# ruanyyyyyyy/point-cloud-process

Hardware: AMD Instinct MI355X
Metric: correspondence-pairs/sec + ms/ICP-iter, 120k-pt KITTI pair (higher is better)
Workload: dtype f64; 1 GPU; point-to-point ICP iteration, 120000 x 120000 KITTI-shaped synthetic scan pair per GPU (BASELINE configs[1]); exact 1-NN via grid; nn=grid, pairs_per_gpu=1, points_src=120000, points_tgt=120000

## Files before the change

### point-cloud-process_amd/csrc/pcr_grid_search.hip

```cpp
#include <atomic>
#include <chrono>
#include <cmath>
#include <cstdlib>
#include <cstring>
#include "pcr_descent.h"
#include "pcr_icp_step.h"

constexpr unsigned int HARD_SCAN_T = 192;
constexpr int HARD_STACK = 160;
constexpr long long ID_NONE = 0x7fffffffffffffffll;
constexpr int H_NLIST = 32;
constexpr int H_CSTRIDE = 32;
__host__ __device__ static inline unsigned int hard_list_cap(long long nq) {
    const long long halves = (nq + 15) / 16;
    return (unsigned int)(((halves + H_NLIST - 1) / H_NLIST) * 16 + 64);
}

template <int G>
__device__ static inline void group_best(double& bd2, long long& bid, unsigned int& bpos) {
#pragma unroll
    for (int off = G / 2; off > 0; off >>= 1) {
        const double od2 = __shfl_xor(bd2, off, 64);
        const long long oid = __shfl_xor(bid, off, 64);
        const unsigned int opos = __shfl_xor(bpos, off, 64);
// ... 33 lines not shown
    unsigned int c_start[WT_MAXC];
    unsigned int c_off[WT_MAXC + 1];
    unsigned short own[WT_PR];
};

__device__ static inline unsigned int wave_incl_scan_max(unsigned int v) {
    v = max(v, dpp_u32<0x111, 0xf>(0u, v));
    v = max(v, dpp_u32<0x112, 0xf>(0u, v));
    v = max(v, dpp_u32<0x114, 0xf>(0u, v));
    v = max(v, dpp_u32<0x118, 0xf>(0u, v));
    v = max(v, dpp_u32<0x142, 0xa>(0u, v));
    v = max(v, dpp_u32<0x143, 0xc>(0u, v));
    return v;
}

__device__ static inline int row16_min(int v) {
    v = min(v, __builtin_amdgcn_update_dpp(0, v, 0xb1, 0xf, 0xf, true));
    v = min(v, __builtin_amdgcn_update_dpp(0, v, 0x4e, 0xf, 0xf, true));
    v = min(v, __builtin_amdgcn_update_dpp(0, v, 0x141, 0xf, 0xf, true));
    v = min(v, __builtin_amdgcn_update_dpp(0, v, 0x140, 0xf, 0xf, true));
    return v;
}
__device__ static inline int row16_max(int v) {
    v = max(v, __builtin_amdgcn_update_dpp(0, v, 0xb1, 0xf, 0xf, true));
    v = max(v, __builtin_amdgcn_update_dpp(0, v, 0x4e, 0xf, 0xf, true));
    v = max(v, __builtin_amdgcn_update_dpp(0, v, 0x141, 0xf, 0xf, true));
    v = max(v, __builtin_amdgcn_update_dpp(0, v, 0x140, 0xf, 0xf, true));
    return v;
}

struct wt_xyz { double x, y, z; };

__device__ static inline wt_xyz ld_xyz_global(const void* p) {
    const __attribute__((address_space(1))) double* g = (const __attribute__((address_space(1))) double*)reinterpret_cast<const double*>(p);
    return wt_xyz{g[0], g[1], g[2]};
}

template <typename T>
__device__ static inline const T* as_global(const T* p) {
    return (const T*)(const __attribute__((address_space(1))) T*)p;
}

struct wt_state {
    double ax, ay, az;
    long long qi;
    float bound2;
    unsigned int cand_pos;
    unsigned int won;
    bool open, clamped, qvalid;
    unsigned int staged;
    unsigned long long dbg_pairs;
    unsigned int dbg_passes;
    unsigned long long probe;
};

struct wt_pre {
    pcr_pt p;
    unsigned int seed_pos;
    wt_xyz seed_b;
};
__device__ __forceinline__ static void wtile_preload(const unsigned int tile, const int lane, const pcr_pt* __restrict__ q, const long long nq,
                                                     const unsigned int* __restrict__ res_pos, const wt_xyz* __restrict__ prev_xyz, wt_pre& P) {
    const long long qi = (long long)tile * WT_Q + (lane & (WT_Q - 1));
    P.seed_pos = POS_NONE;
    P.seed_b = wt_xyz{0.0, 0.0, 0.0};
    P.p.x = P.p.y = P.p.z = 0.0; P.p.id = 0;
    if (qi < nq) {
        if (prev_xyz) {
            P.seed_pos = res_pos[qi];
            P.seed_b = prev_xyz[qi];
        }
        P.p = q[qi];
    }
}

#ifndef PCR_WT_WAVES
#define PCR_WT_WAVES 4
#endif
__device__ __forceinline__ static void wtile_search(const pcr_grid_view& gv, wtile_lds* L, const unsigned int tile, const int lane, const wt_pre& P,
                                                    pcr_pt* __restrict__ q, const long long nq, const pcr_xform& x, const int has_x, const int write_back,
                                                    const double max_d2, const int gated, const unsigned int pcap, unsigned int* __restrict__ res_pos,
                                                    double* __restrict__ res_d2, unsigned long long* __restrict__ dbg,
                                                    const wt_xyz* __restrict__ prev_xyz, wt_state& S, const unsigned long long* probe_p = nullptr,
                                                    const unsigned int probe_stride = 0, const unsigned int probe_groups = 0, const unsigned int probe_total = 0) {
    typedef float f4 __attribute__((ext_vector_type(4)));
    const pcr_pt* __restrict__ g_pts = as_global(gv.pts);
#ifdef PCR_WT_DIAG
    const unsigned long long t_start = dbg ? __builtin_amdgcn_s_memtime() : 0;
    unsigned long long t_ph[8] = {0, 0, 0, 0, 0, 0, 0, 0}, t_last = t_start;
#define WT_STAMP(i) do { if (dbg) { const unsigned long long t_now = __builtin_amdgcn_s_memtime(); t_ph[i] += t_now - t_last; t_last = t_now; } } while (0)
#define WT_WHY(v) do { why = (v); } while (0)
    int why = 0;
#else
#define WT_STAMP(i) do {} while (0)
#define WT_WHY(v) do {} while (0)
#endif
    const long long qi = (long long)tile * WT_Q + (lane & (WT_Q - 1));
    const bool qvalid = qi < nq;
    double ax = 0, ay = 0, az = 0;
    bool clamped = false;
    const unsigned int seed_pos = P.seed_pos;
    const wt_xyz seed_b = P.seed_b;
    if (qvalid) {
        const pcr_pt p = P.p;
        ax = p.x; ay = p.y; az = p.z;
        if (has_x) {
            xform_apply(x, p, &ax, &ay, &az);
            if (write_back && lane < WT_Q) {
                pcr_pt o;
                o.x = ax; o.y = ay; o.z = az; o.id = p.id;
                q[qi] = o;
            }
        }
        cell_coord(ax, gv.lo[0], gv.inv_cell0, &clamped);
        cell_coord(ay, gv.lo[1], gv.inv_cell0, &clamped);
        cell_coord(az, gv.lo[2], gv.inv_cell0, &clamped);
    }
    
    WT_STAMP(0);
    bool open = qvalid;
    const float gate2 = gated ? (float)max_d2 * (1.0f + 1e-6f) : INFINITY;
    float bound2 = gate2;
    unsigned int cand_pos = POS_NONE, won = POS_NONE;
    if (prev_xyz && qvalid && !clamped) {
        const unsigned int pp = seed_pos;
        if (pp != POS_NONE) {
            const wt_xyz b = seed_b;
            const double dx = ax - b.x, dy = ay - b.y, dz = az - b.z;
            const float up = (float)((dx * dx + dy * dy) + dz * dz) * (1.0f + 2e-7f) + 1e-37f;
            if (up < bound2) { bound2 = up; cand_pos = pp; }
        }
    }
    unsigned long long dbg_pairs = 0, probe_v = 0;
    unsigned int dbg_passes = 0, staged = 0;
    const int max_passes = prev_xyz ? WT_PASSES_SEEDED : WT_PASSES;
    unsigned int staged_done = 0;
    float ring = 1.0f;
#pragma unroll 1
    for (int pass = 0; pass < max_passes; ++pass) {
        const bool part = open && !clamped;
        if (!__any(part)) break;
        if (pass > 0 && staged_done > (unsigned int)WT_HEAVY_STOP) break;
        int mn[3], mx[3];
        {
            const float rho = (cand_pos != POS_NONE) ? sqrtf(bound2) * (1.0f + 1e-6f) : fminf((float)gv.cell0 * ring, sqrtf(gate2));
            const double rc = fmin((double)rho * gv.inv_cell0, 262144.0);
            const double tx = (ax - gv.lo[0]) * gv.inv_cell0, ty = (ay - gv.lo[1]) * gv.inv_cell0, tz = (az - gv.lo[2]) * gv.inv_cell0;
            const int cmax = (int)PCR_COORD_MAX;
            mn[0] = part ? max(0, min(cmax, (int)floor(tx - rc) + (int)PCR_COORD_BIAS)) : 0x7fffffff;
            mx[0] = part ? max(0, min(cmax, (int)floor(tx + rc) + (int)PCR_COORD_BIAS)) : -1;
            mn[1] = part ? max(0, min(cmax, (int)floor(ty - rc) + (int)PCR_COORD_BIAS)) : 0x7fffffff;
            mx[1] = part ? max(0, min(cmax, (int)floor(ty + rc) + (int)PCR_COORD_BIAS)) : -1;
            mn[2] = part ? max(0, min(cmax, (int)floor(tz - rc) + (int)PCR_COORD_BIAS)) : 0x7fffffff;
            mx[2] = part ? max(0, min(cmax, (int)floor(tz + rc) + (int)PCR_COORD_BIAS)) : -1;
        }
#pragma unroll
        for (int k = 0; k < 3; ++k) {
            int lo_k = row16_min(mn[k]), hi_k = row16_max(mx[k]);
            lo_k = min(__builtin_amdgcn_readlane(lo_k, 0), __builtin_amdgcn_readlane(lo_k, 16));
            hi_k = max(__builtin_amdgcn_readlane(hi_k, 0), __builtin_amdgcn_readlane(hi_k, 16));
            mn[k] = __builtin_amdgcn_readfirstlane(lo_k);
            mx[k] = __builtin_amdgcn_readfirstlane(hi_k);
        }
        int level = -1, blo0 = 0, blo1 = 0, blo2 = 0, d0 = 0, d1 = 0, d2 = 0;
        const int n_levels = gv.levels;
        for (int l = 0; l < n_levels; ++l) {
            const int b0 = mn[0] >> (2 * l), b1 = mn[1] >> (2 * l), b2 = mn[2] >> (2 * l);
            const int e0 = (mx[0] >> (2 * l)) - b0 + 1, e1 = (mx[1] >> (2 * l)) - b1 + 1, e2 = (mx[2] >> (2 * l)) - b2 + 1;
            if (e0 > WT_MAXC || e1 > WT_MAXC || e2 > WT_MAXC || e0 * e1 > WT_MAXC || e0 * e1 * e2 > WT_MAXC) continue;
            const int n0 = ((b0 + e0 - 1) >> 1) - (b0 >> 1) + 1, n1 = ((b1 + e1 - 1) >> 1) - (b1 >> 1) + 1, n2 = ((b2 + e2 - 1) >> 1) - (b2 >> 1) + 1;
            if (n0 * n1 * n2 > 64) continue;
            level = l; blo0 = b0; blo1 = b1; blo2 = b2; d0 = e0; d1 = e1; d2 = e2;
            break;
        }
        level = __builtin_amdgcn_readfirstlane(level);
        if (level < 0) { if (part) WT_WHY(1); break; }
        blo0 = __builtin_amdgcn_readfirstlane(blo0); blo1 = __builtin_amdgcn_readfirstlane(blo1); blo2 = __builtin_amdgcn_readfirstlane(blo2);
        d0 = __builtin_amdgcn_readfirstlane(d0); d1 = __builtin_amdgcn_readfirstlane(d1); d2 = __builtin_amdgcn_readfirstlane(d2);
        ++dbg_passes;
        WT_STAMP(1);
        unsigned int ncell = 0;
        bool big_child = false;
        {
            const int lim = (int)(PCR_COORD_MAX >> (2 * level));
            const int bx0 = blo0 >> 1, by0 = blo1 >> 1, bz0 = blo2 >> 1;
            const int nb0 = ((blo0 + d0 - 1) >> 1) - bx0 + 1, nb1 = ((blo1 + d1 - 1) >> 1) - by0 + 1, nb2 = ((blo2 + d2 - 1) >> 1) - bz0 + 1;
            const int nb01 = nb0 * nb1, nblk = nb01 * nb2;
            pcr_block_slot e;
            bool have = false;
            int BX = 0, BY = 0, BZ = 0;
            if (lane < nblk) {
                int iz = (int)((float)lane * __builtin_amdgcn_rcpf((float)nb01));
                iz -= (iz * nb01 > lane);
                iz += ((iz + 1) * nb01 <= lane);
                const int rem = lane - iz * nb01;
                int iy = (int)((float)rem * __builtin_amdgcn_rcpf((float)nb0));
                iy -= (iy * nb0 > rem);
                iy += ((iy + 1) * nb0 <= rem);
                const int ix = rem - iy * nb0;
                BX = bx0 + ix; BY = by0 + iy; BZ = bz0 + iz;
                const int blim = lim >> 1;
                if (BX >= 0 && BY >= 0 && BZ >= 0 && BX <= blim && BY <= blim && BZ <= blim)
                    have = lookup_block(as_global(gv.btable[level]), gv.bmask[level], (unsigned int)BX, (unsigned int)BY, (unsigned int)BZ, &e);
// ... 465 lines not shown
        const double cell = gv.cell0 * (double)(1ll << (2 * top));
        const int b0 = (int)(PCR_COORD_BIAS >> (2 * top));
        bool valid = lane < 8;
        const unsigned int X = b0 + (lane & 1), Y = b0 + ((lane >> 1) & 1), Z = b0 + ((lane >> 2) & 1);
        unsigned int s = 0, e = 0;
        double bdist = 0.0;
        if (valid) {
            bdist = box_dist2(gv, top, cell, X, Y, Z, ax, ay, az);
            valid = bdist <= bound2 && lookup_cell(gv.table[top], gv.mask[top], X, Y, Z, &s, &e);
        }
        hard_disperse(gv, L, sp, lane, valid, s, e, X, Y, Z, top, bdist, ax, ay, az, bd2, bid, bpos, bound2, h_pts, bw);
        ++h_steps;
        hard_drain(gv, L, sp, lane, ax, ay, az, bd2, bid, bpos, bound2, h_steps, h_pts, bw);
    }
    {
        const double m = wave_min_f64(bd2);
        unsigned long long cm = __ballot(bpos != POS_NONE && bd2 == m);
        if (!cm) { bd2 = DBL_MAX; bid = ID_NONE; bpos = POS_NONE; if (win) { win[0] = win[1] = win[2] = 0.0; } return; }
        int wl = (int)__ffsll((long long)cm) - 1;
        cm &= cm - 1;
        if (cm) {
            long long best_id = readlane_i64(bid, wl);
            while (cm) {
                const int l = (int)__ffsll((long long)cm) - 1;
                cm &= cm - 1;
                const long long id_l = readlane_i64(bid, l);
                if (id_l < best_id) { best_id = id_l; wl = l; }
            }
        }
        bd2 = m;
        bid = readlane_i64(bid, wl);
        bpos = (unsigned int)__builtin_amdgcn_readlane((int)bpos, wl);
        if (win) {
#pragma unroll
            for (int k = 0; k < 3; ++k)
                win[k] = readlane_f64(bw[k], wl);
        }
    }
}

__global__ void __launch_bounds__(256)
grid_hard_kernel(pcr_grid_view gv, const work_item* __restrict__ list, const unsigned int* __restrict__ count_p, long long nq, double max_d2, int gated,
                 unsigned int* __restrict__ res_pos, double* __restrict__ res_d2, unsigned long long* __restrict__ dbg,
                 const pcr_icp_dev_state* __restrict__ st) {
    __shared__ hard_lds s_lds[4];
    if (st && st->stop) return;
    const int lane = threadIdx.x & 63, wave = threadIdx.x >> 6;
    hard_lds* L = &s_lds[wave];
    unsigned int l_cnt = lane < H_NLIST ? count_p[H_CSTRIDE * lane] : 0u;
    unsigned int l_inc = l_cnt;
#pragma unroll
    for (int off = 1; off < H_NLIST; off <<= 1) {
        const unsigned int o = __shfl_up(l_inc, off, 64);
        if (lane >= off) l_inc += o;
    }
    const unsigned int count = __shfl(l_inc, H_NLIST - 1, 64);
    const unsigned int l_exc = l_inc - l_cnt;
    const unsigned int l_cap = hard_list_cap(nq);
    for (unsigned int w = blockIdx.x * 4 + wave; w < count; w += gridDim.x * 4) {
        const int hl = (int)__ffsll((long long)__ballot(lane < H_NLIST && l_exc <= w && w < l_exc + l_cnt)) - 1;
        const work_item it = list[(size_t)hl * l_cap + (w - __shfl(l_exc, hl, 64))];
        const unsigned long long h_t0 = dbg ? __builtin_amdgcn_s_memtime() : 0;
        unsigned int h_steps = 0, h_pts = 0;
        int s_level0 = 0;
        double bd2;
        long long bid;
        unsigned int bpos;
        hard_search(gv, L, lane, it.ax, it.ay, it.az, gated ? fmin(it.best_d2, max_d2) : it.best_d2, it.best_pos != POS_NONE, bd2, bid, bpos, h_steps,
                    h_pts, s_level0);
        if (lane == 0) {
            res_pos[it.qi] = bpos;
            if (res_d2) res_d2[it.qi] = bd2;
            if (dbg && w < 60000) {
                dbg[(1 << 17) + w * 4 + 0] = __builtin_amdgcn_s_memtime() - h_t0;
                dbg[(1 << 17) + w * 4 + 1] = ((unsigned long long)h_steps << 32);
                dbg[(1 << 17) + w * 4 + 2] = h_pts;
                dbg[(1 << 17) + w * 4 + 3] = (unsigned long long)(it.best_pos != POS_NONE) | ((unsigned long long)(s_level0 + 1) << 8);
            }
        }
    }
}

constexpr int ACC_SETS = 32;
constexpr int PASS_GROUPS = 32;
constexpr int PASS_SYNC_STRIDE = 32;
constexpr int PASS_SYNC_WORDS = PASS_SYNC_STRIDE * (PASS_GROUPS + 1);
constexpr unsigned long long ITEM_NONE = ~0ull;
constexpr unsigned int POISON_HI = 0xfffffffeu;
__device__ static inline unsigned long long item_poison(unsigned int pass_id) { return ((unsigned long long)POISON_HI << 32) | pass_id; }
#ifndef PCR_PASS_SPIN_LIMIT
#define PCR_PASS_SPIN_LIMIT (1u << 21)
#endif
constexpr unsigned int PASS_SPIN_LIMIT = PCR_PASS_SPIN_LIMIT;
constexpr int Q_BITS = 22;
constexpr unsigned long long Q_MASK = (1ull << Q_BITS) - 1ull;
constexpr long long PASS_MAX_NQ = 1ll << 26;
struct pass_args {
    unsigned long long* items;
    unsigned long long* sync;
    unsigned int cap;
    unsigned long long* acc;
    wt_xyz* prev_xyz;
    double scale, inv_scale;
    pcr_icp_dev_state* st;
    pcr_icp_loop_args la;
    unsigned int* tile_cost;
    unsigned int pass_id;
    unsigned long long* host_block;
    unsigned int notify;
    unsigned int* plog;
};
constexpr int PASS_LOG_WORDS = 3 * PCR_ICP_MAX_LOG + 8;
constexpr size_t HOST_LOG_OFF = (sizeof(pcr_icp_dev_state) + 63) & ~(size_t)63;
constexpr size_t HOST_FLAG_OFF = 8192 - 8;
static_assert(HOST_LOG_OFF + 4 * PASS_LOG_WORDS <= HOST_FLAG_OFF, "state + pass log + flag fit the landing block");
__host__ __device__ static inline unsigned int pass_item_cap(long long nq) {
    const long long tiles = (nq + WT_Q - 1) / WT_Q + 4;
    return (unsigned int)(((tiles + PASS_GROUPS - 1) / PASS_GROUPS) * (WT_Q + 1));
}

__device__ static inline long long to_fixed(double v, double scale) {
    constexpr double BIG = 6755399441055744.0;
    return __double_as_longlong(__builtin_fma(v, scale, BIG)) - __double_as_longlong(BIG);
}

__device__ static inline void acc_fixed_add(unsigned long long* __restrict__ acc, unsigned int set, int lane, double mk, double scale) {
    if (lane < PCR_NMOM - 1 && mk != 0.0)
        atomicAdd(acc + (size_t)(set % ACC_SETS) * PCR_NMOM + lane, (unsigned long long)to_fixed(mk, scale));
}

__device__ static inline void acc_fixed_add_ll(unsigned long long* __restrict__ acc, unsigned int set, int lane, long long v) {
    if (lane < PCR_NMOM - 1 && v != 0) atomicAdd(acc + (size_t)(set % ACC_SETS) * PCR_NMOM + lane, (unsigned long long)v);
}

__device__ static inline unsigned long long ld_dev(const unsigned long long* p) {
    return __hip_atomic_load(p, __ATOMIC_RELAXED, __HIP_MEMORY_SCOPE_AGENT);
}
__device__ static inline void st_dev(unsigned long long* p, unsigned long long v) {
    __hip_atomic_store(p, v, __ATOMIC_RELAXED, __HIP_MEMORY_SCOPE_AGENT);
}

union pass_lds {
    wtile_lds t;
    hard_lds h;
    double xch[WT_Q * (PCR_NMOM - 1)];
    long long xll[WT_Q * (PCR_NMOM - 1)];
};

__device__ __forceinline__ static void pass_serve_item(const pcr_grid_view& gv, pass_lds* L, const int lane, const unsigned long long w, const double max_d2,
                                                       const pass_args& A, unsigned int* __restrict__ res_pos, unsigned long long* __restrict__ dbg,
                                                       const unsigned int dbg_slot, const unsigned long long t_start) {
    const unsigned int w_lo = (unsigned int)w, w_hi = (unsigned int)(w >> 32);
    const double ax = __hiloint2double(__builtin_amdgcn_readlane((int)w_hi, 0), __builtin_amdgcn_readlane((int)w_lo, 0));
    const double ay = __hiloint2double(__builtin_amdgcn_readlane((int)w_hi, 1), __builtin_amdgcn_readlane((int)w_lo, 1));
    const double az = __hiloint2double(__builtin_amdgcn_readlane((int)w_hi, 2), __builtin_amdgcn_readlane((int)w_lo, 2));
    const unsigned int qi = (unsigned int)__builtin_amdgcn_readlane((int)w_lo, 3);
    const float cand_b2 = __uint_as_float((unsigned int)__builtin_amdgcn_readlane((int)w_hi, 3));
    const unsigned long long h_t0 = dbg ? __builtin_amdgcn_s_memtime() : 0;
    unsigned int h_steps = 0, h_pts = 0;
    int s_level0 = 0;
    double bd2;
    long long bid;
    unsigned int bpos;
    const bool have_cand = cand_b2 < INFINITY;
    double win[3];
    hard_search(gv, &L->h, lane, ax, ay, az, have_cand ? fmin((double)cand_b2, max_d2) : max_d2, have_cand, bd2, bid, bpos, h_steps, h_pts, s_level0, win);
    wave_sync();
    if (bpos != POS_NONE) {
        if (lane == 0) {
            pcr_pt b;
            b.x = win[0]; b.y = win[1]; b.z = win[2]; b.id = 0;
            A.prev_xyz[qi] = wt_xyz{b.x, b.y, b.z};
            double m[PCR_NMOM];
#pragma unroll
            for (int k = 0; k < PCR_NMOM; ++k) m[k] = 0.0;
            moments_add(m, gv.origin, ax, ay, az, b, max_d2, 1);
#pragma unroll
            for (int k = 0; k < PCR_NMOM - 1; ++k) L->xch[k] = m[k];
        }
        wave_sync();
        acc_fixed_add(A.acc, qi, lane, lane < PCR_NMOM - 1 ? L->xch[lane] : 0.0, A.scale);
        wave_sync();
    }
    if (lane == 0) {
        res_pos[qi] = bpos;
        if (dbg && dbg_slot < 60000) {
            dbg[(1 << 17) + dbg_slot * 4 + 0] = __builtin_amdgcn_s_memtime() - h_t0;
            dbg[(1 << 17) + dbg_slot * 4 + 1] = ((unsigned long long)h_steps << 32) | (unsigned int)((h_t0 - t_start) >> 4);
            dbg[(1 << 17) + dbg_slot * 4 + 2] = h_pts;
            dbg[(1 << 17) + dbg_slot * 4 + 3] = (unsigned long long)have_cand | ((unsigned long long)(s_level0 + 1) << 8);
        }
    }
}

__device__ __forceinline__ static void pass_finish(const pcr_grid_view& gv, pass_lds* L, const int lane, const pass_args& A, unsigned long long* root,
                                                   unsigned long long* __restrict__ dbg) {
    constexpr int HEAD_WORDS = (int)(pcr::ICP_STATE_HEAD_BYTES / 8);
    static_assert(pcr::ICP_STATE_HEAD_BYTES % 8 == 0 && HEAD_WORDS <= 64, "state head: one word per lane");
    double* const head = L->xch + 32;
    unsigned long long hw = 0, err_w = 0;
    if (lane < HEAD_WORDS) hw = reinterpret_cast<const unsigned long long*>(A.st)[lane];
    if (lane == 63) err_w = ld_dev(root + 16);
    const int mom = lane % PCR_NMOM, part = lane / PCR_NMOM;
    long long sum = 0;
    if (part < 3) {
        constexpr int PER = (ACC_SETS + 2) / 3;
        unsigned long long v[PER];
#pragma unroll
        for (int j = 0; j < PER; ++j) {
            const int set = part + 3 * j;
            v[j] = set < ACC_SETS ? ld_dev(A.acc + (size_t)set * PCR_NMOM + mom) : 0ull;
        }
#pragma unroll
        for (int j = 0; j < PER; ++j) {
            const int set = part + 3 * j;
            if (v[j]) st_dev(A.acc + (size_t)set * PCR_NMOM + mom, 0ull);
            sum += (long long)v[j];
        }
    }
    if (dbg && lane == 0) dbg[(1 << 19) - 4] = __builtin_amdgcn_s_memrealtime();
    sum += __shfl(sum, lane + PCR_NMOM, 64) + __shfl(sum, lane + 2 * PCR_NMOM, 64);
    wave_sync();
    if (dbg && lane == 0) dbg[(1 << 19) - 3] = __builtin_amdgcn_s_memrealtime();
    if (lane < PCR_NMOM) L->xch[lane] = (double)sum * A.inv_scale;
    if (lane < HEAD_WORDS) reinterpret_cast<unsigned long long*>(head)[lane] = hw;
    const bool gave_up = __builtin_amdgcn_readlane((int)(unsigned int)err_w, 63) != 0;
    wave_sync();
    if (lane == 0) {
        pcr_icp_dev_state* hs = reinterpret_cast<pcr_icp_dev_state*>(head);
        if (gave_up) { hs->status = PCR_E_HIP; hs->stop = 1; st_dev(root + 16, 0ull); }
        else pcr::icp_step(hs, L->xch, gv.origin, A.la, A.st->r_diff, A.st->t_diff);
    }
    wave_sync();
    if (dbg && lane == 0) dbg[(1 << 19) - 2] = __builtin_amdgcn_s_memrealtime();
    if (A.plog && lane == 0 && A.pass_id < (unsigned int)PCR_ICP_MAX_LOG) A.plog[A.pass_id] = (unsigned int)__builtin_amdgcn_s_memrealtime();
    if (lane < HEAD_WORDS) reinterpret_cast<unsigned long long*>(A.st)[lane] = reinterpret_cast<const unsigned long long*>(head)[lane];
    if (dbg && lane == 0) dbg[(1 << 19) - 1] = __builtin_amdgcn_s_memrealtime();
    if (A.host_block) {
        const int stop_now = reinterpret_cast<const pcr_icp_dev_state*>(head)->stop;
        if (A.notify || stop_now) {
            asm volatile("s_waitcnt vmcnt(0)" ::: "memory");
            wave_sync();
            constexpr int STATE_WORDS = (int)(sizeof(pcr_icp_dev_state) / 8);
            if (lane < HEAD_WORDS) A.host_block[lane] = reinterpret_cast<const unsigned long long*>(head)[lane];
            for (int w = HEAD_WORDS + lane; w < STATE_WORDS; w += 64) A.host_block[w] = ld_dev(reinterpret_cast<const unsigned long long*>(A.st) + w);
            if (A.plog)
                for (int w = lane; w < PASS_LOG_WORDS / 2; w += 64) A.host_block[HOST_LOG_OFF / 8 + w] = ld_dev(reinterpret_cast<const unsigned long long*>(A.plog) + w);
            __threadfence_system();
            wave_sync();
            if (lane == 0) __hip_atomic_store(A.host_block + HOST_FLAG_OFF / 8, (unsigned long long)A.pass_id + 1ull, __ATOMIC_RELEASE, __HIP_MEMORY_SCOPE_SYSTEM);
        }
    }
}

__device__ __forceinline__ static void tile_set_priority(unsigned int last_cost) {
    const unsigned int lc = (unsigned int)__builtin_amdgcn_readfirstlane((int)last_cost);
    const unsigned int c = lc & 0xffffu, had_open = lc >> 16;
    if (c > 3 * WT_PR) __builtin_amdgcn_s_setprio(3);
    else if (c > 2 * WT_PR) __builtin_amdgcn_s_setprio(2);
    else if (c > WT_PR || had_open) __builtin_amdgcn_s_setprio(1);
}
__device__ __forceinline__ static void tile_record_cost(const wt_state& S, int lane, unsigned int* tile_cost, unsigned int tile) {
    wave_sync();
    __builtin_amdgcn_s_setprio(0);
    const unsigned int n_open = (unsigned int)__popcll(__ballot(S.open && lane < WT_Q));
    if (lane == 0) tile_cost[tile] = (S.staged < 0xffffu ? S.staged : 0xffffu) | (n_open << 16);
}

// ... 35 lines not shown
                                                wt_xyz* prev_xyz, const double& scale, unsigned long long* acc, unsigned int tile) {
    double m[PCR_NMOM];
#pragma unroll
    for (int k = 0; k < PCR_NMOM; ++k) m[k] = 0.0;
    if (nb.proven) {
        if (nb.known) { nb.b.x = P.seed_b.x; nb.b.y = P.seed_b.y; nb.b.z = P.seed_b.z; }
        else prev_xyz[S.qi] = wt_xyz{nb.b.x, nb.b.y, nb.b.z};
        moments_add(m, origin, S.ax, S.ay, S.az, nb.b, max_d2, 1);
    }
    if (lane < WT_Q) {
#pragma unroll
        for (int k = 0; k < PCR_NMOM - 1; ++k) L->xll[lane * (PCR_NMOM - 1) + k] = to_fixed(m[k], scale);
    }
    wave_sync();
    long long tot = 0;
    if (lane < PCR_NMOM - 1) {
#pragma unroll 8
        for (int j = 0; j < WT_Q; ++j) tot += L->xll[j * (PCR_NMOM - 1) + lane];
    }
    acc_fixed_add_ll(acc, tile, lane, tot);
}

struct drain_part {
    unsigned int cnt, exc, total;
};
__device__ __forceinline__ static drain_part drain_partition(const unsigned long long* sync, int lane) {
    static_assert(PASS_GROUPS <= 64, "one group per lane");
    drain_part d;
    d.cnt = lane < PASS_GROUPS ? (unsigned int)(sync[(size_t)PASS_SYNC_STRIDE * lane] & Q_MASK) : 0u;
    d.exc = wave_excl_scan_u32(d.cnt, lane, &d.total);
    return d;
}
__device__ __forceinline__ static unsigned long long drain_take(const drain_part& d, unsigned long long* items, unsigned int cap, unsigned int w_i, int lane) {
    const int grp = (int)__ffsll((long long)__ballot(((lane < PASS_GROUPS) & (d.exc <= w_i)) && w_i < d.exc + d.cnt)) - 1;
    const unsigned int idx = w_i - (unsigned int)__builtin_amdgcn_readlane((int)d.exc, grp);
    unsigned long long* it = items + ((size_t)grp * cap + idx) * 4;
    unsigned long long w = ITEM_NONE;
    if (lane < 4) {
        w = it[lane];
        it[lane] = ITEM_NONE;
    }
    return w;
}

#ifndef PCR_PASS_DIAG
#define PCR_PASS_DIAG 0
#endif
__global__ void __launch_bounds__(256) __attribute__((amdgpu_waves_per_eu(PCR_WT_WAVES, 8)))
grid_pass_kernel(const pcr_grid_view* __restrict__ gvp, pcr_grid_view gv, pcr_pt* __restrict__ q, long long nq, double max_d2, int xcd_remap,
                 unsigned int pcap_arg, unsigned int pcap_busy, unsigned int* __restrict__ res_pos, unsigned long long* __restrict__ dbg_arg, int use_prev, int inline_queue,
                 pass_args A) {
    unsigned long long* const dbg = PCR_PASS_DIAG ? dbg_arg : nullptr;
    __shared__ pass_lds s_lds[4];
    const int lane = threadIdx.x & 63, wave = __builtin_amdgcn_readfirstlane((int)(threadIdx.x >> 6));
    const unsigned int tile = wtile_block(xcd_remap) * 4 + wave;
    wt_pre P;
    wtile_preload(tile, lane, q, nq, res_pos, use_prev ? A.prev_xyz : nullptr, P);
    const unsigned int last_cost = use_prev ? A.tile_cost[tile] : 0u;
    unsigned int pcap = pcap_arg;
    if (pcap_busy > pcap_arg && A.plog) {
        const unsigned int prev_items = A.pass_id > 0 && A.pass_id <= (unsigned int)PCR_ICP_MAX_LOG ? A.plog[2 * PCR_ICP_MAX_LOG + A.pass_id - 1] : 0xffffffffu;
        if ((unsigned long long)prev_items * 16ull > (unsigned long long)nq) pcap = pcap_busy;
        pcap = (unsigned int)__builtin_amdgcn_readfirstlane((int)pcap);
    }
    const pcr_xform x = A.st->x;
    if (A.st->stop) return;
    tile_set_priority(last_cost);
    const unsigned long long t_start = dbg ? __builtin_amdgcn_s_memtime() : 0;
    const unsigned long long rt_start = dbg ? __builtin_amdgcn_s_memrealtime() : 0;
    unsigned long long rt_tile = 0, rt_acc = 0;
    unsigned int n_items = 0, n_polls = 0, n_casfail = 0;
    pass_lds* L = &s_lds[wave];
    const unsigned int n_waves = gridDim.x * 4;
    const unsigned int g = tile % PASS_GROUPS;
    const unsigned int g_tiles = n_waves / PASS_GROUPS + (g < n_waves % PASS_GROUPS ? 1u : 0u);
    unsigned long long* const g_q = A.sync + (size_t)PASS_SYNC_STRIDE * g;
    unsigned long long* const g_started = g_q + 16;
    unsigned long long* const g_ticket = g_q + 17;
    unsigned long long* const items = A.items + (size_t)g * A.cap * 4;
    if (lane == 0) __hip_atomic_fetch_add(g_started, 1ull, __ATOMIC_RELAXED, __HIP_MEMORY_SCOPE_AGENT);
    const unsigned int n_groups = n_waves < (unsigned int)PASS_GROUPS ? n_waves : (unsigned int)PASS_GROUPS;
    wt_state S;
    wtile_search(*gvp, &L->t, tile, lane, P, q, nq, x, 1, 1, max_d2, 1, pcap, res_pos, nullptr, dbg, use_prev ? A.prev_xyz : nullptr, S, inline_queue ? A.sync + 16 : nullptr,
                 (unsigned int)PASS_SYNC_STRIDE, n_groups, n_waves);
    tile_record_cost(S, lane, A.tile_cost, tile);
    if (dbg) rt_tile = __builtin_amdgcn_s_memrealtime();
    tile_nb nb;
    tile_neighbour(gv.pts, S, P, lane, nb);
    bool all_started = false;
    if (inline_queue) {
        all_started = S.probe != 0;
        if (!all_started) {
            unsigned long long sv = 0;
            if (lane < (int)n_groups) sv = ld_dev(A.sync + (size_t)PASS_SYNC_STRIDE * lane + 16);
            const bool ok = lane < (int)n_groups && (unsigned int)sv == n_waves / PASS_GROUPS + ((unsigned int)lane < n_waves % PASS_GROUPS ? 1u : 0u);
            all_started = __ballot(ok) == (n_groups >= 64 ? ~0ull : (1ull << n_groups) - 1ull);
        }
    }
    const bool unres = S.open && lane < WT_Q;
    const unsigned long long um = __ballot(unres);
    unsigned int mine = 0;
    bool have_claim = false;
    unsigned long long own = 0;
    unsigned long long* const root = A.sync + (size_t)PASS_SYNC_STRIDE * PASS_GROUPS;
    {
        unsigned int tg;
        const unsigned long long slot_w = publish_reserve(A.sync, um, unres, lane, g, n_groups, tg);
        asm volatile("" :: "v"(slot_w) : "memory");
        if (lane == 0)
            own = __hip_atomic_fetch_add(g_q, (1ull << (2 * Q_BITS)) | (all_started ? 1ull << Q_BITS : 0ull), __ATOMIC_RELAXED, __HIP_MEMORY_SCOPE_AGENT);
        if (unres) publish_store<true>(A.items, A.cap, tg, slot_w, S, (unsigned int)S.qi);
    }
    tile_fold_moments(L, lane, S, P, nb, gv.origin, max_d2, A.prev_xyz, A.scale, A.acc, tile);
    wave_sync();
    {
        {
            const unsigned int o_lo = (unsigned int)__builtin_amdgcn_readfirstlane((int)(unsigned int)own), o_hi = (unsigned int)__builtin_amdgcn_readfirstlane((int)(unsigned int)(own >> 32));
            own = ((unsigned long long)o_hi << 32) | o_lo;
        }
        if (all_started) {
            have_claim = true;
            mine = (unsigned int)((own >> Q_BITS) & Q_MASK);
        }
        if ((unsigned int)(own >> (2 * Q_BITS)) == g_tiles - 1u && inline_queue) {
            int fin = 0;
            if (lane == 0) fin = __hip_atomic_fetch_add(root + 8, 1ull, __ATOMIC_RELAXED, __HIP_MEMORY_SCOPE_AGENT) == (unsigned long long)(n_groups - 1u) ? 1 : 0;
            if (__builtin_amdgcn_readfirstlane(fin)) {
                if (lane == 0) st_dev(root + 8, 0ull);
                unsigned long long qw = 0;
                if (lane < (int)n_groups) qw = ld_dev(A.sync + (size_t)PASS_SYNC_STRIDE * lane);
                const unsigned int R_l = (unsigned int)(qw & Q_MASK);
                for (unsigned int gg = 0; gg < n_groups; ++gg) {
                    const unsigned int R = (unsigned int)__builtin_amdgcn_readlane((int)R_l, (int)gg);
                    const unsigned int gt = n_waves / PASS_GROUPS + (gg < n_waves % PASS_GROUPS ? 1u : 0u);
                    unsigned long long* const base_g = A.items + (size_t)gg * A.cap * 4;
                    for (unsigned int k = lane; k < gt; k += 64) st_dev(base_g + (size_t)(R + k) * 4 + 3, item_poison(A.pass_id));
                }
            }
        }
    }
    if (dbg) rt_acc = __builtin_amdgcn_s_memrealtime();
    if (dbg && lane == 0) {
        atomicAdd(&dbg[blockIdx.x * 4 + 1], S.dbg_pairs);
        atomicAdd(&dbg[blockIdx.x * 4 + 2], (unsigned long long)S.dbg_passes);
        atomicAdd(&dbg[blockIdx.x * 4 + 3], (unsigned long long)__popcll(um));
        atomicMax(&dbg[blockIdx.x * 4 + 0], __builtin_amdgcn_s_memtime() - t_start);
    }
    if (!inline_queue) return;
    bool failed = false, left_by_poison = false;
    for (;;) {
        if (!have_claim) {
            if (!all_started) {
                unsigned long long sv = 0;
                if (lane < (int)n_groups) sv = ld_dev(A.sync + (size_t)PASS_SYNC_STRIDE * lane + 16);
                const bool ok = lane < (int)n_groups && (unsigned int)sv == n_waves / PASS_GROUPS + ((unsigned int)lane < n_waves % PASS_GROUPS ? 1u : 0u);
                all_started = __ballot(ok) == (n_groups >= 64 ? ~0ull : (1ull << n_groups) - 1ull);
            }
            if (all_started) {
                unsigned long long old = 0;
                if (lane == 0) old = __hip_atomic_fetch_add(g_q, 1ull << Q_BITS, __ATOMIC_RELAXED, __HIP_MEMORY_SCOPE_AGENT);
                const unsigned int o_lo = (unsigned int)__builtin_amdgcn_readfirstlane((int)(unsigned int)old), o_hi = (unsigned int)__builtin_amdgcn_readfirstlane((int)(unsigned int)(old >> 32));
                old = ((unsigned long long)o_hi << 32) | o_lo;
                mine = (unsigned int)((old >> Q_BITS) & Q_MASK);
            } else {
                unsigned long long qw = 0;
                if (lane == 0) qw = ld_dev(g_q);
                const unsigned int q_lo = (unsigned int)__builtin_amdgcn_readfirstlane((int)(unsigned int)qw), q_hi = (unsigned int)__builtin_amdgcn_readfirstlane((int)(unsigned int)(qw >> 32));
// ... 205 lines not shown
        }
    }
#pragma unroll
    for (int k = 0; k < PCR_NMOM - 1; ++k) m[k] = wave_total_f64(m[k]);
    const int wave = threadIdx.x >> 6, lane = threadIdx.x & 63;
    if (lane == 63) {
#pragma unroll
        for (int k = 0; k < PCR_NMOM; ++k) s_part[wave][k] = m[k];
    }
    __syncthreads();
    if (threadIdx.x < PCR_NMOM) {
        const double v = (s_part[0][threadIdx.x] + s_part[1][threadIdx.x]) + (s_part[2][threadIdx.x] + s_part[3][threadIdx.x]);
        partials[(long long)blockIdx.x * PCR_NMOM + threadIdx.x] = v;
    }
    if (ticket == nullptr) {
        if (blockIdx.x == 0 && threadIdx.x < H_NLIST) hard_count[H_CSTRIDE * threadIdx.x] = 0;
        return;
    }
    __shared__ unsigned int s_last;
    asm volatile("s_waitcnt vmcnt(0)" ::: "memory");
    __syncthreads();
    if (threadIdx.x == 0) {
        __builtin_amdgcn_fence(__ATOMIC_RELEASE, "agent");
        asm volatile("s_waitcnt vmcnt(0)" ::: "memory");
        const unsigned int t = __hip_atomic_fetch_add(ticket, 1u, __ATOMIC_RELAXED, __HIP_MEMORY_SCOPE_AGENT);
        s_last = (t == gridDim.x - 1) ? 1u : 0u;
        if (s_last) {
            __builtin_amdgcn_fence(__ATOMIC_ACQUIRE, "agent");
            asm volatile("s_waitcnt vmcnt(0)" ::: "memory");
            *ticket = 0;
        }
    }
    __syncthreads();
    if (!s_last) return;
    if (threadIdx.x < H_NLIST) hard_count[H_CSTRIDE * threadIdx.x] = 0;
    __shared__ double s_red[8][32];
    const int k = threadIdx.x & 31, slice = threadIdx.x >> 5;
    double v = 0.0;
    if (k < PCR_NMOM) {
        for (int b0 = slice; b0 < (int)gridDim.x; b0 += 64) {
            double t[8];
#pragma unroll
            for (int u = 0; u < 8; ++u) {
                const int b = b0 + 8 * u;
                t[u] = b < (int)gridDim.x ? partials[(long long)b * PCR_NMOM + k] : 0.0;
            }
#pragma unroll
            for (int u = 0; u < 8; ++u) v += t[u];
        }
    }
    s_red[slice][k] = v;
    __syncthreads();
    __shared__ double s_m[PCR_NMOM];
    if (slice == 0 && k < PCR_NMOM) {
        const double tot = ((s_red[0][k] + s_red[1][k]) + (s_red[2][k] + s_red[3][k])) + ((s_red[4][k] + s_red[5][k]) + (s_red[6][k] + s_red[7][k]));
        if (out) out[k] = tot;
        s_m[k] = tot;
    }
    if (st) {
        __syncthreads();
        if (threadIdx.x == 0) pcr::icp_step(st, s_m, gv.origin, la, st->r_diff, st->t_diff);
    }
}

struct grid_scratch {
    pcr_dev_block res_pos, res_d2;
    pcr_dev_block hard_list;
    pcr_dev_block prev_xyz;
    pcr_dev_block acc, items, tile_cost;
    unsigned int* const hard_count;
    explicit grid_scratch(pcr_ctx* ctx)
        : res_pos(ctx), res_d2(ctx), hard_list(ctx), prev_xyz(ctx), acc(ctx), items(ctx), tile_cost(ctx), hard_count(ctx->d_counters + PCR_HARD_COUNTERS) {}
};

static int grid_scratch_alloc(grid_scratch* sc, int64_t nq, bool want_d2, bool want_hard) {
    int rc;
    if ((rc = sc->res_pos.alloc(sizeof(unsigned int) * nq))) return rc;
    if (want_d2 && (rc = sc->res_d2.alloc(sizeof(double) * nq))) return rc;
    if (want_hard && (rc = sc->hard_list.alloc(sizeof(work_item) * (size_t)H_NLIST * hard_list_cap(nq)))) return rc;
    return PCR_OK;
}

struct pass_layout {
    size_t sync_word, log_word, zero_words;
    unsigned int cap;
    unsigned long long item_words;
};
static pass_layout pass_scratch_layout(long long nq, int n_pairs, bool with_log) {
    pass_layout l;
    l.sync_word = (size_t)n_pairs * ACC_SETS * PCR_NMOM;
    l.log_word = l.sync_word + PASS_SYNC_WORDS;
    l.zero_words = l.log_word + (with_log ? PASS_LOG_WORDS / 2 : 0);
    l.cap = pass_item_cap(nq);
    l.item_words = 4ull * PASS_GROUPS * l.cap;
    return l;
}

static int wtile_blocks(int64_t nq) { return (int)((nq + 4 * WT_Q - 1) / (4 * WT_Q)); }
static int queue_blocks(const pcr_ctx* ctx, long long want) { return (int)(want < 8ll * ctx->cu_count ? (want < 1 ? 1 : want) : 8ll * ctx->cu_count); }

static unsigned int wtile_point_cap(const pcr_ctx* ctx, int64_t nq) {
    const int nblocks = (int)((nq + 63) / 64);
    return (unsigned int)WT_PR * (nblocks > 8 * ctx->cu_count ? WT_ROUNDS_LARGE : WT_ROUNDS_SMALL);
}
constexpr unsigned int WT_BUSY_CAP = WT_PR * 48;
constexpr int WT_XCD_REMAP = 1;

static int grid_search_enqueue(pcr_ctx* ctx, const pcr_index* idx, pcr_pt* q, int64_t nq, hipStream_t stream, const pcr_xform* x, int write_back,
                               double max_d2, bool gated, bool mark, const grid_scratch* sc, const pcr_icp_dev_state* st, bool use_prev = false) {
    const int nblocks = (int)((nq + 63) / 64);
    pcr_xform xi;
    pcr_xform_from_T(nullptr, &xi);
    if (mark) pcr_prof_mark(ctx, 0);
    {
        if (ctx->d_debug) hipMemsetAsync(ctx->d_debug, 0, sizeof(unsigned long long) * ((1 << 16) + 8 * (size_t)nblocks), stream);
        hipLaunchKernelGGL(grid_wtile_kernel, dim3(wtile_blocks(nq)), dim3(256), 0, stream, (const pcr_grid_view*)idx->d_view, q, (long long)nq, x ? *x : xi,
                           (x || st) ? 1 : 0, write_back, max_d2, gated ? 1 : 0, WT_XCD_REMAP, wtile_point_cap(ctx, nq), sc->res_pos.as<unsigned int>(),
                           sc->res_d2.as<double>(), sc->hard_list.as<work_item>(), sc->hard_count, ctx->d_debug, st, (const wt_xyz*)(use_prev ? sc->prev_xyz.p : nullptr));
    }
    if (mark) pcr_prof_mark(ctx, 1);
    hipLaunchKernelGGL(grid_hard_kernel, dim3(queue_blocks(ctx, (nq + 3) / 4)), dim3(256), 0, stream, idx->view, (const work_item*)sc->hard_list.p,
                       (const unsigned int*)sc->hard_count, (long long)nq, max_d2, gated ? 1 : 0, sc->res_pos.as<unsigned int>(), sc->res_d2.as<double>(),
                       ctx->d_debug, st);
    PCR_HIP(ctx, hipGetLastError());
    return PCR_OK;
}

int pcr_grid_nn1(pcr_ctx* ctx, const pcr_index* idx, pcr_cloud* qc, const pcr_xform* x, double max_d2, int32_t* d_idx, double* d_d2) {
    const bool gated = (max_d2 > 0) && std::isfinite(max_d2);
    int rc = pcr_cloud_morton_sort(ctx, qc, idx->cell);
    if (rc) return rc;
    const int64_t nq = qc->n;
    grid_scratch sc(ctx);
    if ((rc = grid_scratch_alloc(&sc, nq, true, true)) || (rc = grid_search_enqueue(ctx, idx, qc->d, nq, ctx->stream, x, 0, max_d2, gated, true, &sc, nullptr)))
        return rc;
    const int grid = (int)((nq + 255) / 256);
    hipLaunchKernelGGL(grid_finalize_nn1_kernel, dim3(grid), dim3(256), 0, ctx->stream, idx->view, (const pcr_pt*)qc->d, (long long)nq,
                       (const unsigned int*)sc.res_pos.p, (const double*)sc.res_d2.p, max_d2, gated ? 1 : 0, d_idx, d_d2, sc.hard_count);
    PCR_HIP(ctx, hipGetLastError());
    return PCR_OK;
}

int pcr_grid_icp_pass(pcr_ctx* ctx, const pcr_index* idx, pcr_cloud* qc, const pcr_xform* x, double max_d2, int write_back,
                      double* d_moments) {
    const bool gated = (max_d2 > 0) && std::isfinite(max_d2);
    int rc = pcr_cloud_morton_sort(ctx, qc, idx->cell);
    if (rc) return rc;
    const int64_t nq = qc->n;
    grid_scratch sc(ctx);
    if ((rc = grid_scratch_alloc(&sc, nq, false, true)) || (rc = grid_search_enqueue(ctx, idx, qc->d, nq, ctx->stream, x, write_back, max_d2, gated, true, &sc, nullptr)))
        return rc;
    int grid = (int)((nq + 1023) / 1024);
    if (grid > ctx->cu_count) grid = ctx->cu_count;
    if ((rc = pcr_ensure_scratch(ctx, sizeof(double) * PCR_NMOM * (size_t)grid))) return rc;
    pcr_prof_mark(ctx, 2);
    hipLaunchKernelGGL(grid_accumulate_kernel, dim3(grid), dim3(256), 0, ctx->stream, idx->view, (const pcr_pt*)qc->d, (long long)nq, *x,
                       write_back ? 0 : 1, (const unsigned int*)sc.res_pos.p, max_d2, gated ? 1 : 0, ctx->d_partials, pcr_counter(ctx, PCR_CW_ICP_TICKET),
                       d_moments, sc.hard_count, (pcr_icp_dev_state*)nullptr, pcr_icp_loop_args{}, (wt_xyz*)nullptr);
    pcr_prof_mark(ctx, 3);
    pcr_prof_mark(ctx, 4);
    PCR_HIP(ctx, hipGetLastError());
    pcr_prof_finish(ctx);
    return PCR_OK;
}

__device__ static inline void pass_fill(unsigned long long* __restrict__ ones_p, unsigned long long ones_n, unsigned long long* __restrict__ zero_p,
                                        unsigned long long zero_n) {
    const unsigned long long stride = (unsigned long long)gridDim.x * blockDim.x, t0 = (unsigned long long)blockIdx.x * blockDim.x + threadIdx.x;
    for (unsigned long long i = t0; i < ones_n; i += stride) ones_p[i] = ~0ull;
    for (unsigned long long i = t0; i < zero_n; i += stride) zero_p[i] = 0ull;
}
__device__ static inline void block_state_from_T0(pcr_icp_dev_state* __restrict__ st, const double* T0) {
    static_assert(sizeof(pcr_icp_dev_state) % 8 == 0, "state in 8-byte words");
    unsigned long long* w = reinterpret_cast<unsigned long long*>(st);
    for (unsigned int i = threadIdx.x; i < sizeof(pcr_icp_dev_state) / 8; i += blockDim.x) w[i] = 0ull;
    __syncthreads();
    if (threadIdx.x == 0) pcr::icp_state_from_T0(T0, st);
}

struct pass_T0 { double v[16]; };
__global__ void __launch_bounds__(256)
pass_init_kernel(unsigned long long* __restrict__ zero_p, unsigned int zero_n, unsigned long long* __restrict__ ones_p, unsigned long long ones_n,
                 pcr_icp_dev_state* __restrict__ st, pass_T0 T0, unsigned int* __restrict__ plog, unsigned long long* __restrict__ host_started) {
    if (host_started && blockIdx.x == 0 && threadIdx.x == 0) __hip_atomic_store(host_started, 1ull, __ATOMIC_RELAXED, __HIP_MEMORY_SCOPE_SYSTEM);
    pass_fill(ones_p, ones_n, zero_p, zero_n);
    if (blockIdx.x != 0) return;
    block_state_from_T0(st, T0.v);
    if (plog && threadIdx.x == 0) plog[3 * PCR_ICP_MAX_LOG] = (unsigned int)__builtin_amdgcn_s_memrealtime();
}

bool pcr_pass_fixed_scale(const double lo[3], const double hi[3], long long nq, double max_d2, double* scale, double* inv_scale) {
    double r2 = 0.0;
    for (int k = 0; k < 3; ++k) r2 += 0.25 * (hi[k] - lo[k]) * (hi[k] - lo[k]);
    const double R = sqrt(r2) + sqrt(max_d2);
    const double M = (double)nq * fmax(fmax(R * R, max_d2), 1.0);
    int ex = 0;
    frexp(M, &ex);
    int exq = 0;
    frexp(M / (double)nq, &exq);
    const int F = (61 - ex < 51 - exq) ? 61 - ex : 51 - exq;
    if (!(M > 0) || !std::isfinite(M) || F < 20) return false;
    *scale = ldexp(1.0, F);
    *inv_scale = ldexp(1.0, -F);
    return true;
}

static std::atomic<int> g_loops_in_flight[64];
struct loop_guard {
    std::atomic<int>& n;
    explicit loop_guard(int device) : n(g_loops_in_flight[(unsigned int)device % 64u]) { n.fetch_add(1); }
    ~loop_guard() { n.fetch_sub(1); }
};

int pcr_grid_icp_loop(pcr_ctx* ctx, const pcr_index* idx, pcr_cloud* qc, const pcr_icp_params* params, const double T0[16],
                      pcr_icp_result* res) {
    const loop_guard in_flight(ctx->device);
    const auto h_t0 = std::chrono::steady_clock::now();
    auto h_us = [&](std::chrono::steady_clock::time_point a) { return std::chrono::duration_cast<std::chrono::nanoseconds>(std::chrono::steady_clock::now() - a).count() / 1e3; };
    for (double& v : ctx->pass_host_us) v = 0.0;
    const char* const wait_s = getenv("PCR_PASS_INLINE");
    const int wait_env = wait_s ? atoi(wait_s) : -1;
    const bool gated = (params->max_d2 > 0) && std::isfinite(params->max_d2);
    int rc = pcr_cloud_morton_sort(ctx, qc, idx->cell);
    if (rc) return rc;
    const int64_t nq = qc->n;
    int grid = (int)((nq + 1023) / 1024);
    if (grid > ctx->cu_count) grid = ctx->cu_count;
    double sc_f = 0, sc_i = 0;
    const bool fused = gated && nq <= PASS_MAX_NQ && getenv("PCR_ICP_NO_FUSED") == nullptr &&
                       pcr_pass_fixed_scale(idx->lo, idx->hi, nq, params->max_d2, &sc_f, &sc_i);
    grid_scratch sc(ctx);
    pcr_dev_block st_blk(ctx);
    if ((rc = grid_scratch_alloc(&sc, nq, false, !fused)) || (rc = sc.prev_xyz.alloc(24 * (size_t)nq))) return rc;
    const pass_layout pl = pass_scratch_layout(nq, 1, true);
    pass_args pa{};
    if (fused) {
        if ((rc = sc.acc.alloc(8 * pl.zero_words)) || (rc = sc.tile_cost.alloc(sizeof(unsigned int) * 4 * (size_t)wtile_blocks(nq))) ||
            (rc = sc.items.alloc(8 * pl.item_words)))
            return rc;
        pa.cap = pl.cap;
        pa.items = sc.items.as<unsigned long long>();
        pa.tile_cost = sc.tile_cost.as<unsigned int>();
        pa.acc = sc.acc.as<unsigned long long>();
        pa.sync = pa.acc + pl.sync_word;
        pa.plog = (unsigned int*)(pa.acc + pl.log_word);
        pa.prev_xyz = sc.prev_xyz.as<wt_xyz>();
        pa.scale = sc_f;
        pa.inv_scale = sc_i;
    }
    if ((rc = pcr_ensure_scratch(ctx, sizeof(double) * PCR_NMOM * (size_t)grid)) || (rc = st_blk.alloc(sizeof(pcr_icp_dev_state)))) return rc;
    pcr_icp_dev_state* const d_st = st_blk.as<pcr_icp_dev_state>();
    static_assert(sizeof(pcr_icp_dev_state) <= 8192, "state must fit the pinned staging buffer");
    pcr_icp_dev_state* h_st = (pcr_icp_dev_state*)ctx->h_state;
    memset(h_st, 0, sizeof(*h_st));
    pcr::icp_state_from_T0(T0, h_st);
    const pcr_icp_loop_args la = pcr_icp_loop_args_from(params);
    volatile unsigned long long* const h_flag = (volatile unsigned long long*)((char*)ctx->h_state + HOST_FLAG_OFF);
    if (fused) {
        void* dp = nullptr;
        if (hipHostGetDevicePointer(&dp, ctx->h_state, 0) == hipSuccess) pa.host_block = (unsigned long long*)dp;
        *h_flag = 0ull;
        h_flag[-1] = 0ull;
    }
    hipError_t e = hipSuccess;
    ctx->pass_host_us[0] = h_us(h_t0);
    if (fused) {
        pass_T0 t0;
        for (int i = 0; i < 16; ++i) t0.v[i] = T0[i];
        const int ib = (int)((pl.item_words + 256 * 8 - 1) / (256 * 8));
        hipLaunchKernelGGL(pass_init_kernel, dim3(ib < 1 ? 1 : (ib > 1024 ? 1024 : ib)), dim3(256), 0, ctx->stream, pa.acc, (unsigned int)pl.zero_words,
                           pa.items, pl.item_words, d_st, t0, pa.plog,
                           pa.host_block ? pa.host_block + HOST_FLAG_OFF / 8 - 1 : (unsigned long long*)nullptr);
        e = hipGetLastError();
    } else e = hipMemcpyAsync(d_st, h_st, sizeof(*h_st), hipMemcpyHostToDevice, ctx->stream);
    pa.st = d_st;
    pa.la = la;
    pcr_xform xi;
    pcr_xform_from_T(nullptr, &xi);
    int enq = 0;
    const double prof_before = ctx->prof_ms[0] + ctx->prof_ms[1] + ctx->prof_ms[2] + ctx->prof_ms[3];
    int chunk = params->min_iter > 2 ? params->min_iter : 2;
    if (ctx->profile) chunk = 1;
    while (e == hipSuccess && rc == PCR_OK && enq < params->max_iter) {
        if (chunk > params->max_iter - enq) chunk = params->max_iter - enq;
        if (chunk > 64) chunk = 64;
        for (int c = 0; c < chunk && rc == PCR_OK; ++c) {
            const bool use_prev = enq + c > 0;
            const bool one_generation = (nq + WT_Q - 1) / WT_Q <= 16ll * ctx->cu_count;
            const int inline_queue = wait_env >= 0 ? wait_env : ((one_generation && !ctx->shared_device && in_flight.n.load(std::memory_order_relaxed) == 1) ? 1 : 0);
            if (fused) {
                if (ctx->profile) pcr_prof_mark(ctx, 0);
                if (ctx->d_debug) hipMemsetAsync(ctx->d_debug, 0, sizeof(unsigned long long) * (inline_queue ? ((1 << 16) + 8 * (size_t)((nq + 63) / 64)) : ((size_t)1 << 19)), ctx->stream);
                pa.pass_id = (unsigned int)(enq + c);
                pa.notify = c == chunk - 1 ? 1u : 0u;
                const unsigned int cap_n = wtile_point_cap(ctx, nq), cap_busy = (!inline_queue && cap_n > (unsigned int)(WT_PR * WT_ROUNDS_SMALL)) ? WT_BUSY_CAP : cap_n;
                hipLaunchKernelGGL(grid_pass_kernel, dim3(wtile_blocks(nq)), dim3(256), 0, ctx->stream, (const pcr_grid_view*)idx->d_view, idx->view, qc->d, (long long)nq,
                                   params->max_d2, WT_XCD_REMAP, cap_n, cap_busy, sc.res_pos.as<unsigned int>(), ctx->d_debug, use_prev ? 1 : 0, inline_queue, pa);
                if (ctx->profile) pcr_prof_mark(ctx, 1);
                if (!inline_queue)
                    hipLaunchKernelGGL(grid_drain_kernel, dim3(queue_blocks(ctx, (nq + 3) / 4)), dim3(256), 0, ctx->stream, idx->view, params->max_d2,
                                       sc.res_pos.as<unsigned int>(), ctx->d_debug, pa);
                if (hipGetLastError() != hipSuccess) { rc = PCR_E_HIP; break; }
                pcr_prof_mark(ctx, 2);
            } else {
                rc = grid_search_enqueue(ctx, idx, qc->d, nq, ctx->stream, nullptr, 1, params->max_d2, gated, ctx->profile, &sc, d_st, use_prev);
                if (rc) break;
                pcr_prof_mark(ctx, 2);
                hipLaunchKernelGGL(grid_accumulate_kernel, dim3(grid), dim3(256), 0, ctx->stream, idx->view, (const pcr_pt*)qc->d, (long long)nq, xi,
                                   0, (const unsigned int*)sc.res_pos.p, params->max_d2, gated ? 1 : 0, ctx->d_partials, pcr_counter(ctx, PCR_CW_ICP_TICKET),
                                   (double*)nullptr, sc.hard_count, d_st, la, sc.prev_xyz.as<wt_xyz>());
            }
            pcr_prof_mark(ctx, 3);
            pcr_prof_mark(ctx, 4);
            pcr_prof_finish(ctx);
        }
        enq += chunk;
        if (rc) break;
        if (ctx->pass_host_us[1] == 0.0) ctx->pass_host_us[1] = h_us(h_t0) - ctx->pass_host_us[0];
        const auto h_tw = std::chrono::steady_clock::now();
        if (pa.host_block) {
            bool seen = false;
            for (unsigned int spins = 0;; ++spins) {
                if (ctx->pass_host_us[4] == 0.0 && h_flag[-1] != 0ull) ctx->pass_host_us[4] = h_us(h_t0);
                const unsigned long long f = __atomic_load_n((const unsigned long long*)h_flag, __ATOMIC_ACQUIRE);
                if (f >= (unsigned long long)enq || (f > 0 && h_st->stop)) { seen = true; break; }
                if ((spins & 255u) == 255u && h_us(h_tw) > 2e6) break;
                __builtin_ia32_pause();
            }
            ctx->pass_host_us[5] = h_us(h_tw);
// ... 177 lines not shown
```

Before: 3.366 billion correspondences/s.

## Carry per-query NN distance lower bounds across ICP passes to skip gated-out queries

Adds per-query lower-bound arrays (gate_est, gate_lb) stored in the fused-pass scratch. When a query has no seed and fails the gate, the hard search runs with a widened radius (kappa 1.25) and records a lower bound on its NN distance. In later passes that bound is reduced by the query's displacement, and if it still exceeds the gate radius the query is skipped without searching. This removes repeated expensive searches for outlier points, in exchange for extra global reads and writes per query and a wider first search.

```diff
diff --git a/point-cloud-process_amd/csrc/pcr_grid_search.hip b/point-cloud-process_amd/csrc/pcr_grid_search.hip
--- a/point-cloud-process_amd/csrc/pcr_grid_search.hip
+++ b/point-cloud-process_amd/csrc/pcr_grid_search.hip
@@ -139,7 +139,9 @@
                                                     const double max_d2, const int gated, const unsigned int pcap, unsigned int* __restrict__ res_pos,
                                                     double* __restrict__ res_d2, unsigned long long* __restrict__ dbg,
                                                     const wt_xyz* __restrict__ prev_xyz, wt_state& S, const unsigned long long* probe_p = nullptr,
-                                                    const unsigned int probe_stride = 0, const unsigned int probe_groups = 0, const unsigned int probe_total = 0) {
+                                                    const unsigned int probe_stride = 0, const unsigned int probe_groups = 0, const unsigned int probe_total = 0,
+                                                    unsigned long long* __restrict__ gate_lb = nullptr, const unsigned long long* __restrict__ gate_est = nullptr,
+                                                    const unsigned int pass_id = 0) {
     typedef float f4 __attribute__((ext_vector_type(4)));
     const pcr_pt* __restrict__ g_pts = as_global(gv.pts);
 #ifdef PCR_WT_DIAG
@@ -156,6 +158,7 @@
     const bool qvalid = qi < nq;
     double ax = 0, ay = 0, az = 0;
     bool clamped = false;
+    bool beyond = false;
     const unsigned int seed_pos = P.seed_pos;
     const wt_xyz seed_b = P.seed_b;
     if (qvalid) {
@@ -173,9 +176,27 @@
         cell_coord(ay, gv.lo[1], gv.inv_cell0, &clamped);
         cell_coord(az, gv.lo[2], gv.inv_cell0, &clamped);
     }
+    if (gate_lb) {
+        const bool lone = qvalid && !clamped && seed_pos == POS_NONE;
+        if (__any(lone)) {
+            float lb = 0.0f;
+            if (lone) {
+                const unsigned long long est = gate_est[qi], own = gate_lb[qi];
+                lb = (unsigned int)(est >> 32) == pass_id ? __uint_as_float((unsigned int)est) : ((unsigned int)(own >> 32) == pass_id ? __uint_as_float((unsigned int)own) : 0.0f);
+            }
+            if (lb > 0.0f) {
+                const double ux = ax - P.p.x, uy = ay - P.p.y, uz = az - P.p.z;
+                const float u2 = (float)((ux * ux + uy * uy) + uz * uz);
+                const float du = sqrtf(u2 * (1.0f + 1e-6f)) * (1.0f + 1e-6f) + 1e-18f;
+                const float nlb = fmaxf((lb - du) * (1.0f - 1e-6f), 0.0f);
+                beyond = gated && nlb > sqrtf((float)max_d2 * (1.0f + 1e-6f)) * (1.0f + 1e-6f);
+                if (lane < WT_Q && nlb > 0.0f) gate_lb[qi] = ((unsigned long long)(pass_id + 1u) << 32) | __float_as_uint(nlb);
+            }
+        }
+    }
     
     WT_STAMP(0);
-    bool open = qvalid;
+    bool open = qvalid && !beyond;
     const float gate2 = gated ? (float)max_d2 * (1.0f + 1e-6f) : INFINITY;
     float bound2 = gate2;
     unsigned int cand_pos = POS_NONE, won = POS_NONE;
@@ -807,6 +828,7 @@
 }
 
 constexpr int ACC_SETS = 32;
+constexpr double GATE_KAPPA = 1.25;
 constexpr int PASS_GROUPS = 32;
 constexpr int PASS_SYNC_STRIDE = 32;
 constexpr int PASS_SYNC_WORDS = PASS_SYNC_STRIDE * (PASS_GROUPS + 1);
@@ -826,6 +848,8 @@
     unsigned int cap;
     unsigned long long* acc;
     wt_xyz* prev_xyz;
+    unsigned long long* gate_lb;
+    unsigned long long* gate_est;
     double scale, inv_scale;
     pcr_icp_dev_state* st;
     pcr_icp_loop_args la;
@@ -888,18 +912,22 @@
     long long bid;
     unsigned int bpos;
     const bool have_cand = cand_b2 < INFINITY;
+    const bool wide = A.gate_est != nullptr && !have_cand;
+    const double wide_d2 = max_d2 * (GATE_KAPPA * GATE_KAPPA);
+    bool inside = false;
     double win[3];
-    hard_search(gv, &L->h, lane, ax, ay, az, have_cand ? fmin((double)cand_b2, max_d2) : max_d2, have_cand, bd2, bid, bpos, h_steps, h_pts, s_level0, win);
+    hard_search(gv, &L->h, lane, ax, ay, az, have_cand ? fmin((double)cand_b2, max_d2) : (wide ? wide_d2 : max_d2), have_cand, bd2, bid, bpos, h_steps, h_pts, s_level0, win);
     wave_sync();
     if (bpos != POS_NONE) {
         if (lane == 0) {
             pcr_pt b;
             b.x = win[0]; b.y = win[1]; b.z = win[2]; b.id = 0;
-            A.prev_xyz[qi] = wt_xyz{b.x, b.y, b.z};
             double m[PCR_NMOM];
 #pragma unroll
             for (int k = 0; k < PCR_NMOM; ++k) m[k] = 0.0;
             moments_add(m, gv.origin, ax, ay, az, b, max_d2, 1);
+            inside = m[0] != 0.0;
+            if (!wide || inside) A.prev_xyz[qi] = wt_xyz{b.x, b.y, b.z};
 #pragma unroll
             for (int k = 0; k < PCR_NMOM - 1; ++k) L->xch[k] = m[k];
         }
@@ -908,7 +936,11 @@
         wave_sync();
     }
     if (lane == 0) {
-        res_pos[qi] = bpos;
+        res_pos[qi] = (wide && !inside) ? POS_NONE : bpos;
+        if (wide) {
+            const float lb = inside ? 0.0f : (float)sqrt(fmin(bd2, wide_d2)) * (1.0f - 1e-6f);
+            A.gate_est[qi] = ((unsigned long long)(A.pass_id + 1u) << 32) | __float_as_uint(lb);
+        }
         if (dbg && dbg_slot < 60000) {
             dbg[(1 << 17) + dbg_slot * 4 + 0] = __builtin_amdgcn_s_memtime() - h_t0;
             dbg[(1 << 17) + dbg_slot * 4 + 1] = ((unsigned long long)h_steps << 32) | (unsigned int)((h_t0 - t_start) >> 4);
@@ -1110,7 +1142,7 @@
     const unsigned int n_groups = n_waves < (unsigned int)PASS_GROUPS ? n_waves : (unsigned int)PASS_GROUPS;
     wt_state S;
     wtile_search(*gvp, &L->t, tile, lane, P, q, nq, x, 1, 1, max_d2, 1, pcap, res_pos, nullptr, dbg, use_prev ? A.prev_xyz : nullptr, S, inline_queue ? A.sync + 16 : nullptr,
-                 (unsigned int)PASS_SYNC_STRIDE, n_groups, n_waves);
+                 (unsigned int)PASS_SYNC_STRIDE, n_groups, n_waves, use_prev ? A.gate_lb : nullptr, A.gate_est, A.pass_id);
     tile_record_cost(S, lane, A.tile_cost, tile);
     if (dbg) rt_tile = __builtin_amdgcn_s_memrealtime();
     tile_nb nb;
@@ -1482,15 +1514,17 @@
 }
 
 struct pass_layout {
-    size_t sync_word, log_word, zero_words;
+    size_t sync_word, log_word, est_word, lb_word, zero_words;
     unsigned int cap;
     unsigned long long item_words;
 };
-static pass_layout pass_scratch_layout(long long nq, int n_pairs, bool with_log) {
+static pass_layout pass_scratch_layout(long long nq, int n_pairs, bool with_log, bool with_bounds = false) {
     pass_layout l;
     l.sync_word = (size_t)n_pairs * ACC_SETS * PCR_NMOM;
     l.log_word = l.sync_word + PASS_SYNC_WORDS;
-    l.zero_words = l.log_word + (with_log ? PASS_LOG_WORDS / 2 : 0);
+    l.est_word = l.log_word + (with_log ? PASS_LOG_WORDS / 2 : 0);
+    l.lb_word = l.est_word + (with_bounds ? (size_t)nq : 0);
+    l.zero_words = l.lb_word + (with_bounds ? (size_t)nq : 0);
     l.cap = pass_item_cap(nq);
     l.item_words = 4ull * PASS_GROUPS * l.cap;
     return l;
@@ -1632,7 +1666,9 @@
     grid_scratch sc(ctx);
     pcr_dev_block st_blk(ctx);
     if ((rc = grid_scratch_alloc(&sc, nq, false, !fused)) || (rc = sc.prev_xyz.alloc(24 * (size_t)nq))) return rc;
-    const pass_layout pl = pass_scratch_layout(nq, 1, true);
+    const char* const lb_s = getenv("PCR_PASS_GATE_LB");
+    const bool gate_bounds = !(lb_s && atoi(lb_s) == 0);
+    const pass_layout pl = pass_scratch_layout(nq, 1, true, gate_bounds);
     pass_args pa{};
     if (fused) {
         if ((rc = sc.acc.alloc(8 * pl.zero_words)) || (rc = sc.tile_cost.alloc(sizeof(unsigned int) * 4 * (size_t)wtile_blocks(nq))) ||
@@ -1645,6 +1681,10 @@
         pa.sync = pa.acc + pl.sync_word;
         pa.plog = (unsigned int*)(pa.acc + pl.log_word);
         pa.prev_xyz = sc.prev_xyz.as<wt_xyz>();
+        if (gate_bounds) {
+            pa.gate_est = pa.acc + pl.est_word;
+            pa.gate_lb = pa.acc + pl.lb_word;
+        }
         pa.scale = sc_f;
         pa.inv_scale = sc_i;
     }
```

Result: faster. 3.416 billion correspondences/s, median of 6 (+1.5%).
